# guxm2021/SVT_SpeechBrain

Hardware: AMD Instinct MI355X
Metric: 10s@16kHz clips/sec encoder+CTC forward, wav2vec2-base, 1/2/4/8 MI355X (higher is better)
Workload: dtype bf16; 1 GPU; wav2vec2-base audio-only AMT forward (encoder + 20-way head + frame decode), 32 x 10 s @16 kHz mono clips per GPU; global_batch=32, per_gpu_batch=32, samples_per_clip=160000, frames_per_clip=499, parallelism=clips sharded over 1 rank(s), streams=2, inputs=resident in HBM

## Files before the change

### svt_speechbrain_amd/csrc/api.hip

```cpp
#include "../../include/svt_mi355.h"
#include "api.h"
#include "common.h"
#include "host.h"

#include <atomic>
#include <cmath>
#include <cstring>
#include <map>
#include <mutex>
#include <string>
#include <vector>

namespace svt {

int hip_fail(hipError_t e, const char* what, const char* file, int line) {
  set_error(std::string("HIP error ") + hipGetErrorName(e) + " (" + hipGetErrorString(e) + ") at " + file + ":" +
          std::to_string(line) + " in " + what);
  return SVT_ERR_HIP;
}

struct ProfState {
  bool on = false;
  int every = 1;
  unsigned tick = 0;
// ... 464 lines not shown
  else if (key == 15) g_stamp_ends = value;
  else if (key == 16) {  }
  else if (key == 18) {  }
  else if (key == 19) g_x3_pairs = value;
  else if (key == 20) g_ln_two_rows = value;
  else if (key == 21) {
    if (value != 0 && value != 3) { set_error("svt_debug_set(21): the attention A/B arms are retired"); return SVT_ERR_INVALID; }
  }
  else if (key == 22) g_conv0_mfma = value;
  else if (key == 23) g_conv3x3_c64 = value;
  else if (key == 24) return g_conv3x3_c64_launches;
  else if (key == 25) g_conv3x3_c64_form = value;
  else if (key == 26) g_stem_pool_fused = value;
  else if (key == 27) g_conv_down_fused = value;
  else if (key == 28) {
    if (value != 0) { set_error("svt_debug_set(28): the two-slot schedule is retired"); return SVT_ERR_INVALID; }
  }
  else if (key == 29) g_gemm_p1w = value;
  else if (key == 30) {
#ifndef SVT_DIAG
    if (value != 0) { set_error("svt_debug_set(30): gemm_p1x_kernel is built by `make DIAG=1` only"); return SVT_ERR_INVALID; }
#endif
    g_gemm_p1x = value;
  }
  else if (key == 31) return g_dev_frees.load(std::memory_order_relaxed);
  else if (key == 32) return set_ticket_fenced(value);
  else if (key == 33) g_gemm_skinny_small_tiles = value;
  else if (key == 34) g_gemm_walk = value;
  else if (key == 35) g_conv_kperm = value;
  else if (key == 36) g_ffn2_ksplit = value;
  else if (key == 37) { if (value < 8 || value > 256 || value % 8) { set_error("svt_debug_set(37): 8 .. 256, a multiple of 8"); return SVT_ERR_INVALID; } g_gemm_persist_wgs = value; }
  else if (key == 38) return g_flash_kernel_id;
  else if (key == 39) return g_gemm_kernel_id;
  else { set_error("svt_debug_set: unknown key"); return SVT_ERR_INVALID; }
  return SVT_OK;
}

int svt_debug_alloc(void** out, size_t bytes, int device) {
  if (!out) { set_error("svt_debug_alloc: null argument"); return SVT_ERR_INVALID; }
  if (int r = check_device(device)) return r;
  SVT_HIP(hipSetDevice(device));
  return dev_alloc(out, bytes);
}
int svt_debug_free(void* p, int device) {
  if (int r = check_device(device)) return r;
  SVT_HIP(hipSetDevice(device));
  dev_free(p);
  return SVT_OK;
}

int svt_debug_clock(int64_t* out_dev, int device, void* stream) {
  if (!out_dev) { set_error("svt_debug_clock: null argument"); return SVT_ERR_INVALID; }
  SVT_HIP(hipSetDevice(device));
  return launch_clock_stamp((long long*)out_dev, (hipStream_t)stream) ? SVT_ERR_HIP : SVT_OK;
}

int svt_prof_enable(int on) { g_prof.on = on != 0; g_prof.every = on > 1 ? on : 1; g_prof.tick = 0; return SVT_OK; }
int svt_prof_reset(void) {
  g_prof.used = 0;
  for (int k = 0; k < 3; ++k) g_prof.flops[k] = g_prof.bytes[k] = 0;
  return SVT_OK;
}
int svt_prof_read(int kind, int64_t* launches, double* total_ms, double* total_flops, double* total_bytes) {
  if (kind < 0 || kind > 2) { set_error("svt_prof_read: kind must be 0..2"); return SVT_ERR_INVALID; }
  double ms = 0;
  int64_t n = 0;
// ... 17 lines not shown
```

### svt_speechbrain_amd/csrc/api_encoder.hip

```cpp
#include "../../include/svt_mi355.h"
#include "api.h"
#include "common.h"
#include "host.h"

#include <cmath>
#include <cstring>
#include <string>
#include <vector>

using namespace svt;

int svt::g_conv_ln_bf16 = 1;

struct ConvLayerW {
  DevBuf w;
  DevBuf w_kperm;
  DevBuf bias;
  DevBuf gamma, beta;
};
struct EncLayerW {
  DevBuf wqkv, bqkv, wo, bo, ln1g, ln1b, w1, b1, w2, b2, ln2g, ln2b;
  DevBuf g_wab, g_bab, g_const;
};

struct svt_encoder {
  svt_encoder_config cfg;
  int device = 0;
  bool finalized = false;
  bool uploaded = false;
  ParamMap params;
  std::vector<ConvLayerW> conv;
  DevBuf fp_g, fp_b, proj_w, proj_b, pos_w, pos_b, enc_g, enc_b;
  DevBuf pos_bn_sc, pos_bn_sh;
  DevBuf pos_wP, pos_bP;
  int pos_P = 0;
  std::vector<DevBuf> pos_ws, pos_bs;
  DevBuf rel_embed;
  DevBuf ones, zeros;
  std::vector<EncLayerW> layers;
  svt_norm_reduce_fn reduce_fn = nullptr;
  void* reduce_user = nullptr;
  int64_t reduce_global_clips = 0;
};

static bool reduced_mode(const svt_encoder_config& c) { return c.precision != SVT_PREC_FP32; }
// ... 595 lines not shown
  const svt_encoder_config& c = x.c;
  const EncWs& w = x.w;
  const int C = x.p.C, D = x.p.D, rows = (int)x.p.rows, pk = x.pk_front;
  const void* proj_in = w.act[cur];
  if (c.feat_proj_layer_norm) {
    LnArgs n = ln_f32(x, w.act[cur], rows, C, x.e->fp_g, x.e->fp_b, c.layer_norm_eps);
    n.x_is_f32 = x.p.sp ? 0 : 1;
    (pk ? n.yP : n.yT) = w.xln; n.pair_kind = pk;
    if (int r = launch_layernorm(n, x.s)) return r;
    proj_in = w.xln;
  }
  GemmArgs g;
  g.A = proj_in; g.W = x.e->proj_w.p; g.C = w.hF; g.bias = x.e->proj_b.as<float>();
  g.M = rows; g.N = D; g.K = C; g.a_rpb = rows; g.a_rstride = C; g.ldw = C; g.ldc = D; g.out_f32 = 1;
  g.a_pairs = pk ? 1 : 0;
  return launch_gemm(x.p.gp, g, x.s);
}

GemmArgs posconv_gemm(const EncRun& x, const DevBuf& W, const DevBuf& bias) {
  const int T = (int)x.p.T, D = x.p.D, G = x.c.pos_conv_groups, cg = D / G, kp = x.c.pos_conv_kernel;
  GemmArgs g;
  g.A = x.w.posg; g.W = W.p; g.C = x.w.preF; g.bias = bias.as<float>();
  g.M = T; g.N = cg; g.K = kp * cg;
  g.a_rpb = T; g.a_rstride = cg;
  g.ldw = g.K; g.ldc = D;
  g.nz = x.p.B * G; g.nz2 = G;
  g.a_z1 = (long)G * (T + kp) * cg; g.a_z2 = (long)(T + kp) * cg;
  g.w_z1 = 0; g.w_z2 = (long)cg * g.K;
  g.c_z1 = (long)T * D; g.c_z2 = cg; g.bias_z2 = cg;
  g.out_f32 = 1;
  return g;
}

int positional_conv(const EncRun& x) {
  const svt_encoder_config& c = x.c;
  const svt_encoder* e = x.e;
  const EncWs& w = x.w;
  const int prec = x.p.sp, gp = x.p.gp, B = x.p.B, T = (int)x.p.T, D = x.p.D, kp = c.pos_conv_kernel, G = c.pos_conv_groups, cg = D / G;
  const float* bn_sc = c.pos_conv_batch_norm ? e->pos_bn_sc.as<float>() : nullptr;
  const float* bn_sh = c.pos_conv_batch_norm ? e->pos_bn_sh.as<float>() : nullptr;
  if (c.pos_conv_depth > 1) {
    const float* cur = w.hF;
    float* lnout = w.xF;
    for (int i = 0; i < c.pos_conv_depth; ++i) {
      if (int r = launch_posconv_gather(prec, cur, B, T, D, G, kp, T + kp, w.posg, x.s)) return r;
      GemmArgs g = posconv_gemm(x, e->pos_ws[i], e->pos_bs[i]);
      g.act = ACT_NONE;
      if (int r = launch_gemm(gp, g, x.s)) return r;
      LnArgs n = ln_f32(x, w.preF, x.p.rows, D, e->ones, e->zeros, 1e-5f);
      n.gelu = 1; n.yF = lnout;
      if (int r = launch_layernorm(n, x.s)) return r;
      cur = lnout;
    }
    return launch_add_f32(w.hF, cur, w.preF, x.p.rows * (int64_t)D, x.s);
  }
  if (x.p.pos_multi) {
    const int Pf = x.p.Pf, Tq = (int)x.p.pos_Tq, Tp = (int)x.p.pos_Tp;
    if (int r = launch_posconv_gather(prec, w.hF, B, T, D, G, kp, Tp, w.posg, x.s, bn_sc, bn_sh)) return r;
    GemmArgs g;
    g.A = w.posg; g.W = e->pos_wP.p; g.C = w.posy; g.bias = e->pos_bP.as<float>();
    g.M = B * Tq; g.N = Pf * cg; g.K = (kp + Pf - 1) * cg;
    g.a_rpb = Tq; g.a_bstride = (long)G * Tp * cg; g.a_rstride = (long)Pf * cg;
    g.ldw = g.K; g.ldc = g.N;
    g.nz = G; g.nz2 = G;
    g.a_z2 = (long)Tp * cg; g.w_z2 = (long)g.N * g.K; g.c_z2 = (long)B * Tq * g.N; g.bias_z2 = g.N;
    g.act = ACT_GELU; g.out_f32 = 0;
    if (int r = launch_gemm(gp, g, x.s)) return r;
    return launch_posconv_scatter_add(w.hF, w.posy, B, T, D, G, Pf, Tq, w.preF, x.s, prec ? 0 : 1);
  }
  if (int r = launch_posconv_gather(prec, w.hF, B, T, D, G, kp, T + kp, w.posg, x.s, bn_sc, bn_sh)) return r;
  GemmArgs g = posconv_gemm(x, e->pos_w, e->pos_b);
  g.resid = w.hF; g.act = ACT_GELU;
  return launch_gemm(gp, g, x.s);
}

struct LayerForm {
  int branch_f32 = 1;
  int ffn1_f32 = 0;
  int ffn1_pairs = 0;
  bool ffn2_ksplit = false;
};

int rows_gemm(const EncRun& x, const void* A, int K, const DevBuf& W, const DevBuf& bias, int N, void* Cout, int out_f32, int act,
              unsigned short* planes = nullptr, int c_pairs = 0) {
  const int rows = (int)x.p.rows;
  GemmArgs g;
  g.A = A; g.W = W.p; g.C = Cout; g.bias = bias.as<float>();
  g.M = rows; g.N = N; g.K = K; g.a_rpb = rows; g.a_rstride = K; g.ldw = K; g.ldc = N;
  g.out_f32 = out_f32; g.act = act;
  g.planes = planes; g.plane_stride = (long)rows * N;
  g.a_pairs = x.pk_enc ? 1 : 0; g.c_pairs = c_pairs;
  return launch_gemm(x.p.gp, g, x.s);
}

int attention_block(const EncRun& x, const EncLayerW& Lw, const LayerForm& f) {
  const EncPlan& p = x.p;
  const EncWs& w = x.w;
  const int D = p.D;
  if (int r = rows_gemm(x, w.xb, D, Lw.wqkv, Lw.bqkv, 3 * D, w.qkv, 0, ACT_NONE, p.planes ? (unsigned short*)w.ab.pl_qkv : nullptr)) return r;
  const float* gate = nullptr;
// ... 21 lines not shown

template <class Ln0, class Ln>
int post_ln_layers(const EncRun& x, const LayerForm& f, Ln0&& ln0, Ln&& ln) {
  if (int r = ln0()) return r;
  for (int l = 0; l < x.c.num_layers; ++l) {
    const EncLayerW& Lw = x.e->layers[l];
    if (int r = attention_block(x, Lw, f)) return r;
    if (int r = ln(Lw, false, false)) return r;
    if (int r = ffn_block(x, Lw, f)) return r;
    if (int r = ln(Lw, true, l + 1 == x.c.num_layers)) return r;
  }
  return SVT_OK;
}

bool ffn2_ksplit_ok(const EncRun& x) {
  const int D = x.p.D, F = x.p.F, rows = (int)x.p.rows;
  if (!(g_ffn2_ksplit && x.w.ksplit && x.p.gp == 1 && F % 256 == 0 && F >= 2048 && g_ln_two_rows)) return false;
  GemmArgs g;
  g.A = x.w.ffn; g.W = x.e->layers[0].w2.p; g.C = x.w.hF; g.M = rows; g.N = D; g.K = F; g.a_rpb = rows; g.a_rstride = F; g.ldw = F; g.ldc = D;
  return g_gemm_skinny && gemm_skinny_eligible(g) && (long)((x.p.rows + 31) / 32) * (D / 32) <= 256;
}

int post_ln_hilo(const EncRun& x) {
  const EncWs& w = x.w;
  const int64_t rows = x.p.rows;
  const int D = x.p.D;
  const float eps = x.c.layer_norm_eps;
  bf16_t* const xh = (bf16_t*)w.xb;
  bf16_t* const xl = (bf16_t*)w.xlo;
  LayerForm f;
  f.branch_f32 = 0;
  f.ffn2_ksplit = ffn2_ksplit_ok(x);
  return post_ln_layers(x, f,
    [&] { return launch_layernorm_hilo(nullptr, nullptr, nullptr, w.preF, rows, D, x.e->enc_g.as<float>(), x.e->enc_b.as<float>(), eps, xh, xl, nullptr, x.s); },
    [&](const EncLayerW& Lw, bool second, bool last) {
      const float *g = (second ? Lw.ln2g : Lw.ln1g).as<float>(), *b = (second ? Lw.ln2b : Lw.ln1b).as<float>();
      float* const yF = last ? x.resid : nullptr;
      if (second && f.ffn2_ksplit)
        return launch_layernorm_hilo_parts(w.ksplit, 4, (long)rows * D, Lw.b2.as<float>(), xh, xl, rows, D, g, b, eps, xh, xl, yF, x.s);
      return launch_layernorm_hilo((const bf16_t*)w.hF, xh, xl, nullptr, rows, D, g, b, eps, xh, xl, yF, x.s);
    });
}

int post_ln_pairs(const EncRun& x) {
  const EncWs& w = x.w;
  const bool pair_resid = x.pk_enc == 3;
  LayerForm f;
  f.branch_f32 = 1; f.ffn1_f32 = 1; f.ffn1_pairs = 1;
  return post_ln_layers(x, f,
    [&] {
      LnArgs n = ln_f32(x, w.preF, x.p.rows, x.p.D, x.e->enc_g, x.e->enc_b, x.c.layer_norm_eps);
      n.yP = w.xb; n.pair_kind = x.pk_enc; n.yF = pair_resid ? nullptr : x.resid;
      return launch_layernorm(n, x.s);
    },
    [&](const EncLayerW& Lw, bool second, bool last) {
      LnArgs n = ln_f32(x, w.hF, x.p.rows, x.p.D, second ? Lw.ln2g : Lw.ln1g, second ? Lw.ln2b : Lw.ln1b, x.c.layer_norm_eps);
      n.yP = w.xb; n.pair_kind = x.pk_enc;
      if (pair_resid) { n.addP = w.xb; n.yF = last ? x.resid : nullptr; }
      else { n.add = x.resid; n.yF = x.resid; }
      return launch_layernorm(n, x.s);
    });
}

int post_ln_plain(const EncRun& x, int branch_f32) {
  const EncWs& w = x.w;
  LayerForm f;
  f.branch_f32 = branch_f32;
  auto out = [&](LnArgs n) { n.yT = w.xb; n.yF = x.p.sp ? x.resid : nullptr; return launch_layernorm(n, x.s); };
  return post_ln_layers(x, f,
    [&] { return out(ln_f32(x, w.preF, x.p.rows, x.p.D, x.e->enc_g, x.e->enc_b, x.c.layer_norm_eps)); },
    [&](const EncLayerW& Lw, bool second, bool) {
      LnArgs n = ln_f32(x, w.hF, x.p.rows, x.p.D, second ? Lw.ln2g : Lw.ln1g, second ? Lw.ln2b : Lw.ln1b, x.c.layer_norm_eps);
      n.x_is_f32 = branch_f32; n.add = x.resid;
// ... 137 lines not shown
```

### svt_speechbrain_amd/csrc/common.h

```cpp
#pragma once
#include <hip/hip_runtime.h>
#include <stdint.h>
#include <string>

typedef __bf16 real_bf16x8 __attribute__((ext_vector_type(8)));
#ifdef SVT_OPERAND_F16
typedef _Float16 bf16_t;
#define SVT_MFMA_16x16x32(a, b, c) __builtin_amdgcn_mfma_f32_16x16x32_f16(a, b, c, 0, 0, 0)
#define SVT_MFMA_32x32x16(a, b, c) __builtin_amdgcn_mfma_f32_32x32x16_f16(a, b, c, 0, 0, 0)
#else
typedef __bf16 bf16_t;
#define SVT_MFMA_16x16x32(a, b, c) __builtin_amdgcn_mfma_f32_16x16x32_bf16(a, b, c, 0, 0, 0)
#define SVT_MFMA_32x32x16(a, b, c) __builtin_amdgcn_mfma_f32_32x32x16_bf16(a, b, c, 0, 0, 0)
#endif
typedef bf16_t bf16x8 __attribute__((ext_vector_type(8)));
typedef bf16_t bf16x4 __attribute__((ext_vector_type(4)));
typedef float f32x4 __attribute__((ext_vector_type(4)));

namespace svt {

#if defined(__HIPCC__)
__device__ __forceinline__ float gelu_fast(float x) {
  const float z = fabsf(x) * 0.70710678118654752440f;
  const float t = __builtin_amdgcn_rcpf(fmaf(0.3275911f, z, 1.0f));
// ... 210 lines not shown

__device__ __forceinline__ void tile_walk(int logical, int tiles_m, int tiles_n, int pm, int& tile_m, int& tile_n) {
  if (pm <= 0) { tile_n = logical % tiles_n; tile_m = logical / tiles_n; return; }
  const int per_panel = pm * tiles_n;
  const int pnl = logical / per_panel, rem = logical - pnl * per_panel;
  const int rows = min(pm, tiles_m - pnl * pm);
  tile_n = rem / rows;
  tile_m = pnl * pm + (rem - tile_n * rows);
}

extern int g_gemm_dbg;
extern int g_gemm_force_bm;
extern int g_gemm_ring;
extern int g_gemm_variant;
extern int g_gemm_skinny;
extern int g_gemm_skinny_max_tiles;
extern int g_gemm_x3;
extern int g_stamp_ends;
extern int g_x3_pairs;
extern int g_gemm_p1w;
extern int g_gemm_p1x;
extern int g_gemm_skinny_small_tiles;
extern int g_gemm_walk;
extern int g_conv_kperm;
extern int g_gemm_persist_wgs;
extern int g_gemm_kernel_id;

extern int g_ln_two_rows;
extern int g_flash_wide;
extern int g_flash_kernel_id;
extern int g_ffn2_ksplit;
#pragma GCC visibility push(hidden)
extern int g_conv_ln_bf16;
extern int g_debug_keep_split;
extern int g_conv_down_fused;
#pragma GCC visibility pop

int ensure_dyn_lds(const void* kernel, int bytes);

int dev_alloc(void** out, size_t bytes);
void dev_free(void* p);
extern int g_guard_alloc;

void prof_begin(hipStream_t s);
void prof_end(hipStream_t s, double flops, double bytes, int kind = 1);

int set_ticket_fenced(int on);
int launch_moments(const float* x, int64_t n, double* moments, void* scratch, int groups_max, hipStream_t s, int groups = 1);
size_t moments_scratch_bytes(int groups_max);
int launch_global_norm(const float* x, float* y, int64_t n, const double* moments, float eps, hipStream_t s, int groups = 1,
                       double n_stat = 0);
int launch_conv0_window_moments(const float* wav, int B, int64_t L, int k, int stride, int64_t T1,
                                double* wm , void* scratch , hipStream_t s);
size_t conv0_window_moments_scratch_bytes(int B, int64_t T1);
int launch_conv0_group_coef(const double* wav_moments , int64_t n_wav, const double* wm, int B,
                            int64_t T1, int C, int k, const float* w0 , const float* b0 ,
                            const float* gamma, const float* beta, float eps_wav, float eps_gn,
                            float* coef , hipStream_t s, int clips_per_norm_group);
struct FrameOut { float p_on, p_off; int32_t octave, pitch_class; };
int launch_head_fused(const float* x, int64_t rows, int K, const float* w, const float* wsum, const float* b, int N, float* dots,
                      double* mom, int64_t rows_per_group, float eps, float* logits, FrameOut* frames, int n_oct, int n_cls,
                      hipStream_t s,
                      double n_stat = 0, int (*between)(void*) = nullptr, void* between_arg = nullptr, void* scratch = nullptr);
size_t head_scratch_bytes(int64_t rows, int groups_max);

struct LnArgs {
  int prec = 0;
  const void* x = nullptr;
  int x_is_f32 = 1;
  int64_t rows = 0;
  int D = 0;
  const float* gamma = nullptr;
  const float* beta = nullptr;
  float eps = 1e-5f;
  int gelu = 0;
  void* yT = nullptr;
  float* yF = nullptr;
  const float* add = nullptr;
  float* sumF = nullptr;
  void* yP = nullptr;
  int pair_kind = 0;
  const void* addP = nullptr;
};
int launch_layernorm(const LnArgs& a, hipStream_t s);
bool layernorm_hilo_ok(int D);
int launch_layernorm_hilo_parts(const float* parts, int nparts, long part_stride, const float* pbias, const bf16_t* rh, const bf16_t* rl, int64_t rows,
                                int D, const float* gamma, const float* beta, float eps, bf16_t* yh, bf16_t* yl, float* yF, hipStream_t s);
int launch_layernorm_hilo(const bf16_t* branch, const bf16_t* rh, const bf16_t* rl, const float* x32, int64_t rows, int D,
                          const float* gamma, const float* beta, float eps, bf16_t* yh, bf16_t* yl, float* yF, hipStream_t s);

int launch_conv0_group_apply(int prec, const float* wav, int B, int64_t L, int k, int stride, int64_t T1, int C,
                             const float* coef, void* out , hipStream_t s, int pair_kind = 0);
int launch_conv0_layer(int prec, const float* wav, int B, int64_t L, int k, int stride, int64_t T1, int C,
                       const double* wav_moments, int64_t n_wav, float eps_wav, const float* w0, const float* b0,
                       const float* gamma, const float* beta, float eps, void* out, hipStream_t s, int clips_per_norm_group,
                       int pair_kind = 0);
int launch_f32_to_pairs(int kind, const float* x, void* out, int64_t n, hipStream_t s);
int launch_pairs_to_f32(int kind, const void* in, const void* lo_plane, float* y, int64_t n, hipStream_t s);

bool conv0_mfma_ok(int prec, int pair_kind, int k, int stride, int C);
size_t conv0_mfma_table_bytes(int B);
int launch_conv0_mfma_group(const float* wav, int B, int64_t L, int stride, int64_t T1, const float* coef, void* table_ws, void* out,
                            hipStream_t s, int pair_kind = 0);
int launch_conv0_mfma_layer(const float* wav, int B, int64_t L, int stride, int64_t T1, const double* wav_moments, int64_t n_wav,
                            float eps_wav, const float* w0, const float* b0, const float* gamma, const float* beta, float eps, void* table_ws,
                            void* out, hipStream_t s, int clips_per_norm_group, int pair_kind = 0);
extern int g_conv0_mfma;

int launch_f32_to_bf16(const float* in, bf16_t* out, int64_t n, hipStream_t s);
int launch_zero_bytes(void* p, size_t bytes, hipStream_t s);
int launch_copy_f32(const float* in, float* out, int64_t n, hipStream_t s);
int launch_zero_cols(float* p, int64_t rows, int cols, int64_t ld, hipStream_t s);
int launch_posconv_gather(int prec, const float* h, int B, int T, int D, int G, int kp, int Tp, void* out, hipStream_t s,
                          const float* sc = nullptr, const float* sh = nullptr);
int launch_posconv_scatter_add(const float* h, const void* y, int B, int T, int D, int G, int P, int Tq, float* pre, hipStream_t s,
                               int y_f32 = 0);
int launch_softmax_rows(int prec, const float* S, int64_t rows, int T, int Tp, void* P, hipStream_t s);
int launch_transpose_v(int prec, const void* qkv, int B, int T, int H, int dh, long ld, long voff, int Tp,
                       void* Vt, hipStream_t s);
int launch_axpby(int prec, const void* x, const void* y, float a, float b, void* out, int64_t n, hipStream_t s);
int launch_add_pe(int prec, const float* x, int B, int T, int Tsrc, int D, const float* pe, float* outF, void* outT,
                  hipStream_t s);
// ... 127 lines not shown
```

### svt_speechbrain_amd/csrc/conv0_mfma.hip

```cpp
#include "common.h"

namespace svt {
namespace {

constexpr int K0 = 10, C0 = 512, TBL16 = 2048;

template <int PK> struct C0T { typedef bf16_t piece; };
template <> struct C0T<2> { typedef __bf16 piece; };
template <> struct C0T<3> { typedef _Float16 piece; };
template <int PK> __device__ __forceinline__ f32x4 c0_mma(const typename C0T<PK>::piece __attribute__((ext_vector_type(8))) & a, const uint4& b, const f32x4& c) {
  typedef typename C0T<PK>::piece P;
  typedef P P8 __attribute__((ext_vector_type(8)));
  if constexpr (PK == 3) return __builtin_amdgcn_mfma_f32_16x16x32_f16(a, __builtin_bit_cast(P8, b), c, 0, 0, 0);
  else if constexpr (PK == 2) return __builtin_amdgcn_mfma_f32_16x16x32_bf16(a, __builtin_bit_cast(P8, b), c, 0, 0, 0);
  else return SVT_MFMA_16x16x32(a, __builtin_bit_cast(P8, b), c);
}
template <int PK> __device__ __forceinline__ void c0_store8(void* out, int64_t e, f32x2_t (&p)[4]) {
  typedef typename C0T<PK>::piece P;
  typedef P P8 __attribute__((ext_vector_type(8)));
  if constexpr (PK == 0) {
    gelu_bf16x2_x4(p);
    P8 o;
#pragma unroll
    for (int i = 0; i < 4; ++i) { o[2 * i] = (P)p[i].x; o[2 * i + 1] = (P)p[i].y; }
    *(P8*)((P*)out + e) = o;
  } else {
    P8 hi, lo;
#pragma unroll
    for (int i = 0; i < 4; ++i) {
      const f32x2_t y = gelu_fast2(p[i]);
      hi[2 * i] = (P)y.x; lo[2 * i] = (P)(y.x - (float)hi[2 * i]);
      hi[2 * i + 1] = (P)y.y; lo[2 * i + 1] = (P)(y.y - (float)hi[2 * i + 1]);
    }
    char* d = (char*)out + (e >> 5) * 128 + (e & 31) * 2;
    *(P8*)d = hi;
    *(P8*)(d + 64) = lo;
  }
}

__global__ __launch_bounds__(256) void conv0_coef_exp_kernel(const float* __restrict__ coef, int* __restrict__ exps) {
  const int b = blockIdx.x;
  float mx = 0.f;
  for (int i = threadIdx.x; i < C0 * K0; i += 256) mx = fmaxf(mx, fabsf(coef[((long)b * C0 + i / K0) * (K0 + 1) + i % K0]));
#pragma unroll
  for (int o = 32; o > 0; o >>= 1) mx = fmaxf(mx, __shfl_xor(mx, o, 64));
  __shared__ float part[4];
  if ((threadIdx.x & 63) == 0) part[threadIdx.x >> 6] = mx;
  __syncthreads();
  if (threadIdx.x == 0) {
    mx = fmaxf(fmaxf(part[0], part[1]), fmaxf(part[2], part[3]));
    int e = 0;
    if (mx > 0.f && mx < 3e38f) (void)frexpf(mx, &e);
    exps[b] = e > 100 ? 100 : (e < -100 ? -100 : e);
  }
}

template <int PK>
__global__ void conv0_table_kernel(const float* __restrict__ w, long w_clip_stride, int w_row, const float* __restrict__ bias,
                                   void* __restrict__ table_, const int* __restrict__ tap_exp) {
  typedef typename C0T<PK>::piece bf16_t;
  typedef bf16_t bf16x8 __attribute__((ext_vector_type(8)));
  bf16_t* table = (bf16_t*)table_;
  const int b = blockIdx.y;
  const int idx = blockIdx.x * blockDim.x + threadIdx.x;
  if (idx >= TBL16) return;
  const int blk = idx >> 6, lane = idx & 63, q = blk >> 3, nb = blk & 7, g = lane >> 4, j = lane & 15;
  const int c = 128 * q + 8 * j + nb;
  const float* wc = w + (long)b * w_clip_stride + (long)c * w_row;
  const float bv = bias ? bias[c] : (w_row == K0 + 1 ? wc[K0] : 0.f);
  const float tap_scale = tap_exp ? ldexpf(1.f, -tap_exp[b]) : 1.f;
  bf16x8 o;
#pragma unroll
  for (int i = 0; i < 8; ++i) {
    const int k = 8 * g + i;
    const float src = k < 30 ? wc[k % 10] * tap_scale : bv;
    const bf16_t hi = (bf16_t)src;
    const bf16_t lo = (bf16_t)(src - (float)hi);
    o[i] = (k < 20 || k == 30) ? hi : lo;
  }
  *(bf16x8*)(table + ((long)b * TBL16 + idx) * 8) = o;
}

template <int MODE, int PK = 0>
__global__ __launch_bounds__(256) void conv0_mfma_kernel(const float* __restrict__ wav, int64_t L, int stride, int64_t T1,
                                                         const void* __restrict__ table_, long table_clip_stride,
                                                         const double* __restrict__ wav_mom, int64_t n_wav, float eps_wav,
                                                         const float* __restrict__ gamma, const float* __restrict__ beta, float eps, int cpg,
                                                         void* __restrict__ out, const int* __restrict__ tap_exp) {
  typedef typename C0T<PK>::piece bf16_t;
  typedef bf16_t bf16x8 __attribute__((ext_vector_type(8)));
  const bf16_t* table = (const bf16_t*)table_;
  constexpr int FPW = 64;
  __shared__ __attribute__((aligned(16))) uint4 tbl[TBL16];
  __shared__ float xs[4][FPW * 5 + 16];
  const int tid = threadIdx.x, lane = tid & 63, wave = tid >> 6;
  const int b = blockIdx.y;
  {
    const uint4* tg = (const uint4*)(table + (long)b * table_clip_stride);
    for (int i = tid; i < TBL16; i += 256) tbl[i] = tg[i];
  }
  float mu = 0.f, rn = 1.f, xscale = 1.f, bscale = 1.f;
  if (MODE == 1 && wav_mom) {
    const double* wm = wav_mom + 2 * (b / cpg);
// ... 89 lines not shown
      }
#pragma unroll
      for (int r = 0; r < 4; ++r) {
        float qq = 0.f;
#pragma unroll
        for (int blk = 0; blk < 32; ++blk) { const float d = acc[blk][r] - mean[r]; qq = fmaf(d, d, qq); }
#pragma unroll
        for (int o = 8; o > 0; o >>= 1) qq += __shfl_xor(qq, o, 64);
        rstd[r] = rsqrtf(qq * (1.f / C0) + eps);
      }
#pragma unroll
      for (int q = 0; q < 4; ++q) {
        __builtin_amdgcn_sched_barrier(0);
        const float4 g0 = *(const float4*)(gamma + 128 * q + 8 * j), g1 = *(const float4*)(gamma + 128 * q + 8 * j + 4);
        const float4 b0 = *(const float4*)(beta + 128 * q + 8 * j), b1 = *(const float4*)(beta + 128 * q + 8 * j + 4);
        const float gg[8] = {g0.x, g0.y, g0.z, g0.w, g1.x, g1.y, g1.z, g1.w}, bb[8] = {b0.x, b0.y, b0.z, b0.w, b1.x, b1.y, b1.z, b1.w};
#pragma unroll
        for (int r = 0; r < 4; ++r) {
          f32x2_t p[4];
#pragma unroll
          for (int i = 0; i < 4; ++i)
            p[i] = f32x2_t{fmaf((acc[q * 8 + 2 * i][r] - mean[r]) * rstd[r], gg[2 * i], bb[2 * i]),
                           fmaf((acc[q * 8 + 2 * i + 1][r] - mean[r]) * rstd[r], gg[2 * i + 1], bb[2 * i + 1])};
          if (fr0 + r < nfr) c0_store8<PK>(out, e0 + (int64_t)r * C0 + 128 * q, p);
        }
      }
    }
  }
}

}

int g_conv0_mfma = 1;

bool conv0_mfma_ok(int prec, int pair_kind, int k, int stride, int C) {
  return g_conv0_mfma && (prec == 1 || pair_kind == 2 || pair_kind == 3) && k == K0 && stride >= 1 && stride <= 5 && C == C0;
}
size_t conv0_mfma_table_bytes(int B) { return (size_t)B * TBL16 * 16 + (((size_t)B * 4 + 255) & ~(size_t)255); }

#define SVT_C0_DISPATCH(PKV, STMT)                 \
  if ((PKV) == 3) { constexpr int PK_ = 3; STMT }  \
  else if ((PKV) == 2) { constexpr int PK_ = 2; STMT } \
  else { constexpr int PK_ = 0; STMT }

int launch_conv0_mfma_group(const float* wav, int B, int64_t L, int stride, int64_t T1, const float* coef, void* table_ws, void* out,
                            hipStream_t s, int pair_kind) {
  if (((uintptr_t)table_ws & 15) || ((uintptr_t)out & 127)) { set_error("conv0_mfma: alignment"); return -1; }
  dim3 grid((unsigned)((T1 + 255) / 256), B);
  int* exps = (int*)((char*)table_ws + (size_t)B * TBL16 * 16);
  hipLaunchKernelGGL(conv0_coef_exp_kernel, dim3(B), dim3(256), 0, s, coef, exps);
  SVT_C0_DISPATCH(pair_kind,
    hipLaunchKernelGGL((conv0_table_kernel<PK_>), dim3(TBL16 / 256, B), dim3(256), 0, s, coef, (long)C0 * (K0 + 1), K0 + 1, (const float*)nullptr,
                       table_ws, (const int*)exps);
    hipLaunchKernelGGL((conv0_mfma_kernel<0, PK_>), grid, dim3(256), 0, s, wav, L, stride, T1, (const void*)table_ws, (long)TBL16 * 8,
                       (const double*)nullptr, (int64_t)1, 0.f, (const float*)nullptr, (const float*)nullptr, 0.f, 1, out, (const int*)exps);)
  SVT_LAUNCH_CHECK();
  return 0;
}

int launch_conv0_mfma_layer(const float* wav, int B, int64_t L, int stride, int64_t T1, const double* wav_moments, int64_t n_wav,
                            float eps_wav, const float* w0, const float* b0, const float* gamma, const float* beta, float eps, void* table_ws,
                            void* out, hipStream_t s, int cpg, int pair_kind) {
  if (((uintptr_t)table_ws & 15) || ((uintptr_t)out & 127) || ((uintptr_t)gamma & 15) || ((uintptr_t)beta & 15)) { set_error("conv0_mfma: alignment"); return -1; }
  dim3 grid((unsigned)((T1 + 255) / 256), B);
  SVT_C0_DISPATCH(pair_kind,
    hipLaunchKernelGGL((conv0_table_kernel<PK_>), dim3(TBL16 / 256, 1), dim3(256), 0, s, w0, 0L, K0, b0, table_ws, (const int*)nullptr);
    hipLaunchKernelGGL((conv0_mfma_kernel<1, PK_>), grid, dim3(256), 0, s, wav, L, stride, T1, (const void*)table_ws, 0L, wav_moments, n_wav,
                       eps_wav, gamma, beta, eps, cpg, out, (const int*)nullptr);)
  SVT_LAUNCH_CHECK();
  return 0;
}
#undef SVT_C0_DISPATCH

}
```

### svt_speechbrain_amd/csrc/layernorm.hip

```cpp
#include "device_util.h"
#include <type_traits>

namespace svt {
namespace {
template <typename TI, typename TO>
__global__ __launch_bounds__(256) void layernorm_kernel(const TI* x, const float* add, float* sumF, int64_t rows, int D,
                                                        const float* gamma, const float* beta, float eps, int gelu,
                                                        TO* yT, float* yF) {
  const int lane = threadIdx.x & 63;
  const int64_t row = (int64_t)blockIdx.x * 4 + (threadIdx.x >> 6);
  if (row >= rows) return;
  const TI* xr = x + row * D;
  const float* ar = add ? add + row * D : nullptr;
  float s = 0.f;
  for (int i = lane; i < D; i += 64) s += ld<TI>(xr, i) + (ar ? ar[i] : 0.f);
  const float mean = wave_sum(s) / (float)D;
  float q = 0.f;
  for (int i = lane; i < D; i += 64) { const float d = ld<TI>(xr, i) + (ar ? ar[i] : 0.f) - mean; q += d * d; }
  const float rstd = rsqrtf(wave_sum(q) / (float)D + eps);
  for (int i = lane; i < D; i += 64) {
    const float xv = ld<TI>(xr, i) + (ar ? ar[i] : 0.f);
    if (sumF) sumF[row * D + i] = xv;
    float v = (xv - mean) * rstd * gamma[i] + beta[i];
    if (gelu) v = gelu_erf(v);
// ... 187 lines not shown
                                                             bf16_t* yh, bf16_t* yl, float* yF) {
  constexpr int D = 64 * VPT, NV = VPT / 4;
  const int lane = threadIdx.x & 63;
  const int64_t row = (int64_t)blockIdx.x * 4 + (threadIdx.x >> 6);
  if (row >= rows) return;
  float v[VPT];
  float s = 0.f;
#pragma unroll
  for (int j = 0; j < NV; ++j) {
    const long o = row * D + (lane + 64 * j) * 4;
    const bf16x4 h = *(const bf16x4*)(rh + o), l = *(const bf16x4*)(rl + o);
    float4 t = float4{(float)h[0] + (float)l[0], (float)h[1] + (float)l[1], (float)h[2] + (float)l[2], (float)h[3] + (float)l[3]};
    if (branch) {
      const bf16x4 a = *(const bf16x4*)(branch + o);
      t.x += (float)a[0]; t.y += (float)a[1]; t.z += (float)a[2]; t.w += (float)a[3];
    }
    v[4 * j] = t.x; v[4 * j + 1] = t.y; v[4 * j + 2] = t.z; v[4 * j + 3] = t.w;
    s += (t.x + t.y) + (t.z + t.w);
  }
  const float mean = wave_sum(s) * (1.f / D);
  float q = 0.f;
#pragma unroll
  for (int i = 0; i < VPT; ++i) { v[i] -= mean; q = fmaf(v[i], v[i], q); }
  const float rstd = rsqrtf(wave_sum(q) * (1.f / D) + eps);
#pragma unroll
  for (int j = 0; j < NV; ++j) {
    const int c = (lane + 64 * j) * 4;
    const float4 g = *(const float4*)(gamma + c), b = *(const float4*)(beta + c);
    const float o[4] = {fmaf(v[4 * j] * rstd, g.x, b.x), fmaf(v[4 * j + 1] * rstd, g.y, b.y),
                        fmaf(v[4 * j + 2] * rstd, g.z, b.z), fmaf(v[4 * j + 3] * rstd, g.w, b.w)};
    bf16x4 oh, ol;
#pragma unroll
    for (int i = 0; i < 4; ++i) { oh[i] = (bf16_t)o[i]; ol[i] = (bf16_t)(o[i] - (float)oh[i]); }
    *(bf16x4*)(yh + row * D + c) = oh;
    *(bf16x4*)(yl + row * D + c) = ol;
    if (yF) *(float4*)(yF + row * D + c) = float4{o[0], o[1], o[2], o[3]};
  }
}

template <int D, bool PARTS = false>
__global__ __launch_bounds__(256) void layernorm_hilo2_kernel(const bf16_t* branch, const bf16_t* rh, const bf16_t* rl,
                                                              int64_t rows, const float* gamma, const float* beta, float eps,
                                                              bf16_t* yh, bf16_t* yl, float* yF, const float* parts = nullptr, int nparts = 0,
                                                              long part_stride = 0, const float* pbias = nullptr) {
  constexpr int NC = D / 256;
  const int lane = threadIdx.x & 63, sub = lane & 31;
  const int64_t row = (int64_t)blockIdx.x * 8 + (threadIdx.x >> 6) * 2 + (lane >> 5);
  if (row >= rows) return;
  float v[NC][8];
  float s = 0.f;
#pragma unroll
  for (int j = 0; j < NC; ++j) {
    const long o = row * D + (sub + 32 * j) * 8;
    const bf16x8 h = *(const bf16x8*)(rh + o), l = *(const bf16x8*)(rl + o);
#pragma unroll
    for (int i = 0; i < 8; ++i) v[j][i] = (float)h[i] + (float)l[i];
    if constexpr (PARTS) {
      float a[8];
      {
        const float4 t0 = *(const float4*)(parts + o), t1 = *(const float4*)(parts + o + 4);
        a[0] = t0.x; a[1] = t0.y; a[2] = t0.z; a[3] = t0.w; a[4] = t1.x; a[5] = t1.y; a[6] = t1.z; a[7] = t1.w;
      }
      for (int k = 1; k < nparts; ++k) {
        const float4 t0 = *(const float4*)(parts + k * part_stride + o), t1 = *(const float4*)(parts + k * part_stride + o + 4);
        a[0] += t0.x; a[1] += t0.y; a[2] += t0.z; a[3] += t0.w; a[4] += t1.x; a[5] += t1.y; a[6] += t1.z; a[7] += t1.w;
      }
      const int c = (sub + 32 * j) * 8;
      const float4 b0 = *(const float4*)(pbias + c), b1 = *(const float4*)(pbias + c + 4);
// ... 2 lines not shown
      for (int i = 0; i < 8; ++i) v[j][i] += (float)(bf16_t)(a[i] + bb[i]);
    } else if (branch) {
      const bf16x8 a = *(const bf16x8*)(branch + o);
#pragma unroll
      for (int i = 0; i < 8; ++i) v[j][i] += (float)a[i];
    }
    s += ((v[j][0] + v[j][1]) + (v[j][2] + v[j][3])) + ((v[j][4] + v[j][5]) + (v[j][6] + v[j][7]));
  }
#pragma unroll
  for (int o = 16; o > 0; o >>= 1) s += __shfl_xor(s, o, 64);
  const float mean = s * (1.f / D);
  float q = 0.f;
#pragma unroll
  for (int j = 0; j < NC; ++j)
#pragma unroll
    for (int i = 0; i < 8; ++i) { v[j][i] -= mean; q = fmaf(v[j][i], v[j][i], q); }
#pragma unroll
  for (int o = 16; o > 0; o >>= 1) q += __shfl_xor(q, o, 64);
  const float rstd = rsqrtf(q * (1.f / D) + eps);
#pragma unroll
  for (int j = 0; j < NC; ++j) {
    const int c = (sub + 32 * j) * 8;
    const float4 g0 = *(const float4*)(gamma + c), g1 = *(const float4*)(gamma + c + 4);
    const float4 b0 = *(const float4*)(beta + c), b1 = *(const float4*)(beta + c + 4);
    const float gg[8] = {g0.x, g0.y, g0.z, g0.w, g1.x, g1.y, g1.z, g1.w}, bb[8] = {b0.x, b0.y, b0.z, b0.w, b1.x, b1.y, b1.z, b1.w};
    float o[8];
    bf16x8 oh, ol;
#pragma unroll
    for (int i = 0; i < 8; ++i) {
      o[i] = fmaf(v[j][i] * rstd, gg[i], bb[i]);
      oh[i] = (bf16_t)o[i];
      ol[i] = (bf16_t)(o[i] - (float)oh[i]);
    }
    *(bf16x8*)(yh + row * D + c) = oh;
    *(bf16x8*)(yl + row * D + c) = ol;
    if (yF) {
      *(float4*)(yF + row * D + c) = float4{o[0], o[1], o[2], o[3]};
      *(float4*)(yF + row * D + c + 4) = float4{o[4], o[5], o[6], o[7]};
    }
  }
}
template <int VPT>
__global__ __launch_bounds__(256) void layernorm_f32_to_hilo_kernel(const float* x, int64_t rows, const float* gamma,
                                                                    const float* beta, float eps, bf16_t* yh, bf16_t* yl) {
  constexpr int D = 64 * VPT, NV = VPT / 4;
  const int lane = threadIdx.x & 63;
  const int64_t row = (int64_t)blockIdx.x * 4 + (threadIdx.x >> 6);
  if (row >= rows) return;
  float v[VPT];
  float s = 0.f;
#pragma unroll
  for (int j = 0; j < NV; ++j) {
    const float4 t = ((const float4*)(x + row * D))[lane + 64 * j];
    v[4 * j] = t.x; v[4 * j + 1] = t.y; v[4 * j + 2] = t.z; v[4 * j + 3] = t.w;
    s += (t.x + t.y) + (t.z + t.w);
  }
  const float mean = wave_sum(s) * (1.f / D);
  float q = 0.f;
#pragma unroll
  for (int i = 0; i < VPT; ++i) { v[i] -= mean; q = fmaf(v[i], v[i], q); }
  const float rstd = rsqrtf(wave_sum(q) * (1.f / D) + eps);
#pragma unroll
  for (int j = 0; j < NV; ++j) {
    const int c = (lane + 64 * j) * 4;
    const float4 g = *(const float4*)(gamma + c), b = *(const float4*)(beta + c);
    const float o[4] = {fmaf(v[4 * j] * rstd, g.x, b.x), fmaf(v[4 * j + 1] * rstd, g.y, b.y),
                        fmaf(v[4 * j + 2] * rstd, g.z, b.z), fmaf(v[4 * j + 3] * rstd, g.w, b.w)};
    bf16x4 oh, ol;
#pragma unroll
    for (int i = 0; i < 4; ++i) { oh[i] = (bf16_t)o[i]; ol[i] = (bf16_t)(o[i] - (float)oh[i]); }
    *(bf16x4*)(yh + row * D + c) = oh;
    *(bf16x4*)(yl + row * D + c) = ol;
  }
}
}
bool layernorm_hilo_ok(int D) { return D == 512 || D == 768 || D == 1024; }
int launch_layernorm_hilo_parts(const float* parts, int nparts, long part_stride, const float* pbias, const bf16_t* rh, const bf16_t* rl, int64_t rows,
                                int D, const float* gamma, const float* beta, float eps, bf16_t* yh, bf16_t* yl, float* yF, hipStream_t s) {
  if (!parts || nparts < 1 || !pbias || !(D == 512 || D == 768 || D == 1024) || (part_stride & 3) || !aligned(15, parts, pbias, rh, rl, yh, yl, yF, gamma, beta)) { set_error("layernorm (K-split branch): D in {512, 768, 1024} and 16-byte aligned buffers"); return -1; }
  const dim3 grid2((unsigned)((rows + 7) / 8)), block(256);
  ln_width(D, [&](auto vpt) {
    hipLaunchKernelGGL((layernorm_hilo2_kernel<64 * decltype(vpt)::value, true>), grid2, block, 0, s, nullptr, rh, rl, rows, gamma, beta, eps, yh, yl, yF, parts, nparts, part_stride, pbias);
  });
  SVT_LAUNCH_CHECK();
  return 0;
}
int launch_layernorm_hilo(const bf16_t* branch, const bf16_t* rh, const bf16_t* rl, const float* x32, int64_t rows, int D,
                          const float* gamma, const float* beta, float eps, bf16_t* yh, bf16_t* yl, float* yF, hipStream_t s) {
  const dim3 grid((unsigned)((rows + 3) / 4)), grid2((unsigned)((rows + 7) / 8)), block(256);
  ln_width(D, [&](auto vpt) {
    constexpr int VPT = decltype(vpt)::value;
    if (x32) hipLaunchKernelGGL((layernorm_f32_to_hilo_kernel<VPT>), grid, block, 0, s, x32, rows, gamma, beta, eps, yh, yl);
    else if (g_ln_two_rows && aligned(15, branch, rh, rl, yh, yl, yF, gamma, beta)) hipLaunchKernelGGL((layernorm_hilo2_kernel<64 * VPT>), grid2, block, 0, s, branch, rh, rl, rows, gamma, beta, eps, yh, yl, yF);
    else hipLaunchKernelGGL((layernorm_hilo_kernel<VPT>), grid, block, 0, s, branch, rh, rl, rows, gamma, beta, eps, yh, yl, yF);
  });
  SVT_LAUNCH_CHECK();
  return 0;
}

}
```

Measured before the change: 6315 clips/s.

## Fuse posconv scatter-add into first LayerNorm, skip last-layer planes, fold conv0 exponent

The positional-conv scatter-add and the encoder's first LayerNorm now run as one kernel that reads the residual and the grouped conv output directly, so the fp32 intermediate no longer round-trips through memory. The last encoder LayerNorm can now write only its fp32 result and skip the unused bf16 hi/lo planes. The conv0 per-clip exponent reduction is folded into the table kernel, removing one launch. Each block of the table kernel recomputes the max reduction, which adds some redundant work, and debug counters are added.

```diff
diff --git a/svt_speechbrain_amd/csrc/api.hip b/svt_speechbrain_amd/csrc/api.hip
--- a/svt_speechbrain_amd/csrc/api.hip
+++ b/svt_speechbrain_amd/csrc/api.hip
@@ -520,6 +520,10 @@
   else if (key == 37) { if (value < 8 || value > 256 || value % 8) { set_error("svt_debug_set(37): 8 .. 256, a multiple of 8"); return SVT_ERR_INVALID; } g_gemm_persist_wgs = value; }
   else if (key == 38) return g_flash_kernel_id;
   else if (key == 39) return g_gemm_kernel_id;
+  else if (key == 40) g_posconv_ln_fused = value;
+  else if (key == 41) g_last_ln_f32_only = value;
+  else if (key == 42) g_conv0_self_exp = value;
+  else if (key == 43) { if (value < 0 || value > 2) { set_error("svt_debug_set(43): 0 .. 2"); return SVT_ERR_INVALID; } return g_seam_runs[value]; }
   else { set_error("svt_debug_set: unknown key"); return SVT_ERR_INVALID; }
   return SVT_OK;
 }
diff --git a/svt_speechbrain_amd/csrc/api_encoder.hip b/svt_speechbrain_amd/csrc/api_encoder.hip
--- a/svt_speechbrain_amd/csrc/api_encoder.hip
+++ b/svt_speechbrain_amd/csrc/api_encoder.hip
@@ -11,6 +11,9 @@
 using namespace svt;
 
 int svt::g_conv_ln_bf16 = 1;
+int svt::g_posconv_ln_fused = 1;
+int svt::g_last_ln_f32_only = 1;
+int svt::g_seam_runs[3] = {0, 0, 0};
 
 struct ConvLayerW {
   DevBuf w;
@@ -672,6 +675,13 @@
   return g;
 }
 
+bool posconv_ln_fused(const EncRun& x) {
+  const EncWs& w = x.w;
+  return g_posconv_ln_fused && x.p.hilo && x.p.sp && x.p.pos_multi && x.c.pos_conv_depth <= 1 &&
+         posconv_add_layernorm_hilo_ok(x.p.D, x.c.pos_conv_groups, w.hF, w.posy, x.e->enc_g.as<float>(), x.e->enc_b.as<float>(),
+                                       (const bf16_t*)w.xb, (const bf16_t*)w.xlo);
+}
+
 int positional_conv(const EncRun& x) {
   const svt_encoder_config& c = x.c;
   const svt_encoder* e = x.e;
@@ -706,6 +716,7 @@
     g.a_z2 = (long)Tp * cg; g.w_z2 = (long)g.N * g.K; g.c_z2 = (long)B * Tq * g.N; g.bias_z2 = g.N;
     g.act = ACT_GELU; g.out_f32 = 0;
     if (int r = launch_gemm(gp, g, x.s)) return r;
+    if (posconv_ln_fused(x)) return SVT_OK;
     return launch_posconv_scatter_add(w.hF, w.posy, B, T, D, G, Pf, Tq, w.preF, x.s, prec ? 0 : 1);
   }
   if (int r = launch_posconv_gather(prec, w.hF, B, T, D, G, kp, T + kp, w.posg, x.s, bn_sc, bn_sh)) return r;
@@ -793,13 +804,23 @@
   f.branch_f32 = 0;
   f.ffn2_ksplit = ffn2_ksplit_ok(x);
   return post_ln_layers(x, f,
-    [&] { return launch_layernorm_hilo(nullptr, nullptr, nullptr, w.preF, rows, D, x.e->enc_g.as<float>(), x.e->enc_b.as<float>(), eps, xh, xl, nullptr, x.s); },
+    [&] {
+      if (posconv_ln_fused(x)) {
+        ++g_seam_runs[0];
+        return launch_posconv_add_layernorm_hilo(w.hF, (const bf16_t*)w.posy, x.p.B, (int)x.p.T, D, x.c.pos_conv_groups, x.p.Pf, (int)x.p.pos_Tq,
+                                                 x.e->enc_g.as<float>(), x.e->enc_b.as<float>(), eps, xh, xl, x.s);
+      }
+      return launch_layernorm_hilo(nullptr, nullptr, nullptr, w.preF, rows, D, x.e->enc_g.as<float>(), x.e->enc_b.as<float>(), eps, xh, xl, nullptr, x.s);
+    },
     [&](const EncLayerW& Lw, bool second, bool last) {
       const float *g = (second ? Lw.ln2g : Lw.ln1g).as<float>(), *b = (second ? Lw.ln2b : Lw.ln1b).as<float>();
       float* const yF = last ? x.resid : nullptr;
+      const bool planes = !(last && g_last_ln_f32_only);
+      if (!planes) ++g_seam_runs[1];
+      bf16_t *const yh = planes ? xh : nullptr, *const yl = planes ? xl : nullptr;
       if (second && f.ffn2_ksplit)
-        return launch_layernorm_hilo_parts(w.ksplit, 4, (long)rows * D, Lw.b2.as<float>(), xh, xl, rows, D, g, b, eps, xh, xl, yF, x.s);
-      return launch_layernorm_hilo((const bf16_t*)w.hF, xh, xl, nullptr, rows, D, g, b, eps, xh, xl, yF, x.s);
+        return launch_layernorm_hilo_parts(w.ksplit, 4, (long)rows * D, Lw.b2.as<float>(), xh, xl, rows, D, g, b, eps, yh, yl, yF, x.s);
+      return launch_layernorm_hilo((const bf16_t*)w.hF, xh, xl, nullptr, rows, D, g, b, eps, yh, yl, yF, x.s);
     });
 }
 
diff --git a/svt_speechbrain_amd/csrc/common.h b/svt_speechbrain_amd/csrc/common.h
--- a/svt_speechbrain_amd/csrc/common.h
+++ b/svt_speechbrain_amd/csrc/common.h
@@ -266,6 +266,10 @@
 extern int g_ffn2_ksplit;
 #pragma GCC visibility push(hidden)
 extern int g_conv_ln_bf16;
+extern int g_posconv_ln_fused;
+extern int g_last_ln_f32_only;
+extern int g_conv0_self_exp;
+extern int g_seam_runs[3];
 extern int g_debug_keep_split;
 extern int g_conv_down_fused;
 #pragma GCC visibility pop
@@ -322,6 +326,9 @@
                                 int D, const float* gamma, const float* beta, float eps, bf16_t* yh, bf16_t* yl, float* yF, hipStream_t s);
 int launch_layernorm_hilo(const bf16_t* branch, const bf16_t* rh, const bf16_t* rl, const float* x32, int64_t rows, int D,
                           const float* gamma, const float* beta, float eps, bf16_t* yh, bf16_t* yl, float* yF, hipStream_t s);
+bool posconv_add_layernorm_hilo_ok(int D, int G, const float* h, const void* y, const float* gamma, const float* beta, const bf16_t* yh, const bf16_t* yl);
+int launch_posconv_add_layernorm_hilo(const float* h, const bf16_t* y, int B, int T, int D, int G, int P, int Tq, const float* gamma,
+                                      const float* beta, float eps, bf16_t* yh, bf16_t* yl, hipStream_t s);
 
 int launch_conv0_group_apply(int prec, const float* wav, int B, int64_t L, int k, int stride, int64_t T1, int C,
                              const float* coef, void* out , hipStream_t s, int pair_kind = 0);
diff --git a/svt_speechbrain_amd/csrc/conv0_mfma.hip b/svt_speechbrain_amd/csrc/conv0_mfma.hip
--- a/svt_speechbrain_amd/csrc/conv0_mfma.hip
+++ b/svt_speechbrain_amd/csrc/conv0_mfma.hip
@@ -38,6 +38,11 @@
   }
 }
 
+__device__ __forceinline__ int conv0_tap_exp(float mx) {
+  int e = 0;
+  if (mx > 0.f && mx < 3e38f) (void)frexpf(mx, &e);
+  return e > 100 ? 100 : (e < -100 ? -100 : e);
+}
 __global__ __launch_bounds__(256) void conv0_coef_exp_kernel(const float* __restrict__ coef, int* __restrict__ exps) {
   const int b = blockIdx.x;
   float mx = 0.f;
@@ -47,28 +52,35 @@
   __shared__ float part[4];
   if ((threadIdx.x & 63) == 0) part[threadIdx.x >> 6] = mx;
   __syncthreads();
-  if (threadIdx.x == 0) {
-    mx = fmaxf(fmaxf(part[0], part[1]), fmaxf(part[2], part[3]));
-    int e = 0;
-    if (mx > 0.f && mx < 3e38f) (void)frexpf(mx, &e);
-    exps[b] = e > 100 ? 100 : (e < -100 ? -100 : e);
-  }
+  if (threadIdx.x == 0) exps[b] = conv0_tap_exp(fmaxf(fmaxf(part[0], part[1]), fmaxf(part[2], part[3])));
 }
 
 template <int PK>
 __global__ void conv0_table_kernel(const float* __restrict__ w, long w_clip_stride, int w_row, const float* __restrict__ bias,
-                                   void* __restrict__ table_, const int* __restrict__ tap_exp) {
+                                   void* __restrict__ table_, const int* __restrict__ tap_exp, int* __restrict__ exp_out) {
   typedef typename C0T<PK>::piece bf16_t;
   typedef bf16_t bf16x8 __attribute__((ext_vector_type(8)));
   bf16_t* table = (bf16_t*)table_;
   const int b = blockIdx.y;
+  int own_exp = 0;
+  if (exp_out) {
+    float mx = 0.f;
+    for (int i = threadIdx.x; i < C0 * K0; i += 256) mx = fmaxf(mx, fabsf(w[(long)b * w_clip_stride + (long)(i / K0) * w_row + i % K0]));
+#pragma unroll
+    for (int o = 32; o > 0; o >>= 1) mx = fmaxf(mx, __shfl_xor(mx, o, 64));
+    __shared__ float part[4];
+    if ((threadIdx.x & 63) == 0) part[threadIdx.x >> 6] = mx;
+    __syncthreads();
+    own_exp = conv0_tap_exp(fmaxf(fmaxf(part[0], part[1]), fmaxf(part[2], part[3])));
+    if (blockIdx.x == 0 && threadIdx.x == 0) exp_out[b] = own_exp;
+  }
   const int idx = blockIdx.x * blockDim.x + threadIdx.x;
   if (idx >= TBL16) return;
   const int blk = idx >> 6, lane = idx & 63, q = blk >> 3, nb = blk & 7, g = lane >> 4, j = lane & 15;
   const int c = 128 * q + 8 * j + nb;
   const float* wc = w + (long)b * w_clip_stride + (long)c * w_row;
   const float bv = bias ? bias[c] : (w_row == K0 + 1 ? wc[K0] : 0.f);
-  const float tap_scale = tap_exp ? ldexpf(1.f, -tap_exp[b]) : 1.f;
+  const float tap_scale = exp_out ? ldexpf(1.f, -own_exp) : (tap_exp ? ldexpf(1.f, -tap_exp[b]) : 1.f);
   bf16x8 o;
 #pragma unroll
   for (int i = 0; i < 8; ++i) {
@@ -224,6 +236,7 @@
 }
 
 int g_conv0_mfma = 1;
+int g_conv0_self_exp = 1;
 
 bool conv0_mfma_ok(int prec, int pair_kind, int k, int stride, int C) {
   return g_conv0_mfma && (prec == 1 || pair_kind == 2 || pair_kind == 3) && k == K0 && stride >= 1 && stride <= 5 && C == C0;
@@ -240,10 +253,12 @@
   if (((uintptr_t)table_ws & 15) || ((uintptr_t)out & 127)) { set_error("conv0_mfma: alignment"); return -1; }
   dim3 grid((unsigned)((T1 + 255) / 256), B);
   int* exps = (int*)((char*)table_ws + (size_t)B * TBL16 * 16);
-  hipLaunchKernelGGL(conv0_coef_exp_kernel, dim3(B), dim3(256), 0, s, coef, exps);
+  const bool self_exp = g_conv0_self_exp && pair_kind == 0;
+  if (self_exp) ++g_seam_runs[2];
+  else hipLaunchKernelGGL(conv0_coef_exp_kernel, dim3(B), dim3(256), 0, s, coef, exps);
   SVT_C0_DISPATCH(pair_kind,
     hipLaunchKernelGGL((conv0_table_kernel<PK_>), dim3(TBL16 / 256, B), dim3(256), 0, s, coef, (long)C0 * (K0 + 1), K0 + 1, (const float*)nullptr,
-                       table_ws, (const int*)exps);
+                       table_ws, self_exp ? (const int*)nullptr : (const int*)exps, self_exp ? exps : (int*)nullptr);
     hipLaunchKernelGGL((conv0_mfma_kernel<0, PK_>), grid, dim3(256), 0, s, wav, L, stride, T1, (const void*)table_ws, (long)TBL16 * 8,
                        (const double*)nullptr, (int64_t)1, 0.f, (const float*)nullptr, (const float*)nullptr, 0.f, 1, out, (const int*)exps);)
   SVT_LAUNCH_CHECK();
@@ -256,7 +271,7 @@
   if (((uintptr_t)table_ws & 15) || ((uintptr_t)out & 127) || ((uintptr_t)gamma & 15) || ((uintptr_t)beta & 15)) { set_error("conv0_mfma: alignment"); return -1; }
   dim3 grid((unsigned)((T1 + 255) / 256), B);
   SVT_C0_DISPATCH(pair_kind,
-    hipLaunchKernelGGL((conv0_table_kernel<PK_>), dim3(TBL16 / 256, 1), dim3(256), 0, s, w0, 0L, K0, b0, table_ws, (const int*)nullptr);
+    hipLaunchKernelGGL((conv0_table_kernel<PK_>), dim3(TBL16 / 256, 1), dim3(256), 0, s, w0, 0L, K0, b0, table_ws, (const int*)nullptr, (int*)nullptr);
     hipLaunchKernelGGL((conv0_mfma_kernel<1, PK_>), grid, dim3(256), 0, s, wav, L, stride, T1, (const void*)table_ws, 0L, wav_moments, n_wav,
                        eps_wav, gamma, beta, eps, cpg, out, (const int*)nullptr);)
   SVT_LAUNCH_CHECK();
diff --git a/svt_speechbrain_amd/csrc/layernorm.hip b/svt_speechbrain_amd/csrc/layernorm.hip
--- a/svt_speechbrain_amd/csrc/layernorm.hip
+++ b/svt_speechbrain_amd/csrc/layernorm.hip
@@ -243,8 +243,10 @@
     bf16x4 oh, ol;
 #pragma unroll
     for (int i = 0; i < 4; ++i) { oh[i] = (bf16_t)o[i]; ol[i] = (bf16_t)(o[i] - (float)oh[i]); }
-    *(bf16x4*)(yh + row * D + c) = oh;
-    *(bf16x4*)(yl + row * D + c) = ol;
+    if (yh) {
+      *(bf16x4*)(yh + row * D + c) = oh;
+      *(bf16x4*)(yl + row * D + c) = ol;
+    }
     if (yF) *(float4*)(yF + row * D + c) = float4{o[0], o[1], o[2], o[3]};
   }
 }
@@ -313,12 +315,36 @@
       oh[i] = (bf16_t)o[i];
       ol[i] = (bf16_t)(o[i] - (float)oh[i]);
     }
-    *(bf16x8*)(yh + row * D + c) = oh;
-    *(bf16x8*)(yl + row * D + c) = ol;
+    if (yh) {
+      *(bf16x8*)(yh + row * D + c) = oh;
+      *(bf16x8*)(yl + row * D + c) = ol;
+    }
     if (yF) {
       *(float4*)(yF + row * D + c) = float4{o[0], o[1], o[2], o[3]};
       *(float4*)(yF + row * D + c + 4) = float4{o[4], o[5], o[6], o[7]};
     }
+  }
+}
+template <int VPT>
+__device__ __forceinline__ void row_f32_to_hilo(float (&v)[VPT], float s, int64_t row, int lane, const float* gamma, const float* beta,
+                                                float eps, bf16_t* yh, bf16_t* yl) {
+  constexpr int D = 64 * VPT, NV = VPT / 4;
+  const float mean = wave_sum(s) * (1.f / D);
+  float q = 0.f;
+#pragma unroll
+  for (int i = 0; i < VPT; ++i) { v[i] -= mean; q = fmaf(v[i], v[i], q); }
+  const float rstd = rsqrtf(wave_sum(q) * (1.f / D) + eps);
+#pragma unroll
+  for (int j = 0; j < NV; ++j) {
+    const int c = (lane + 64 * j) * 4;
+    const float4 g = *(const float4*)(gamma + c), b = *(const float4*)(beta + c);
+    const float o[4] = {fmaf(v[4 * j] * rstd, g.x, b.x), fmaf(v[4 * j + 1] * rstd, g.y, b.y),
+                        fmaf(v[4 * j + 2] * rstd, g.z, b.z), fmaf(v[4 * j + 3] * rstd, g.w, b.w)};
+    bf16x4 oh, ol;
+#pragma unroll
+    for (int i = 0; i < 4; ++i) { oh[i] = (bf16_t)o[i]; ol[i] = (bf16_t)(o[i] - (float)oh[i]); }
+    *(bf16x4*)(yh + row * D + c) = oh;
+    *(bf16x4*)(yl + row * D + c) = ol;
   }
 }
 template <int VPT>
@@ -336,29 +362,40 @@
     v[4 * j] = t.x; v[4 * j + 1] = t.y; v[4 * j + 2] = t.z; v[4 * j + 3] = t.w;
     s += (t.x + t.y) + (t.z + t.w);
   }
-  const float mean = wave_sum(s) * (1.f / D);
-  float q = 0.f;
-#pragma unroll
-  for (int i = 0; i < VPT; ++i) { v[i] -= mean; q = fmaf(v[i], v[i], q); }
-  const float rstd = rsqrtf(wave_sum(q) * (1.f / D) + eps);
-#pragma unroll
-  for (int j = 0; j < NV; ++j) {
-    const int c = (lane + 64 * j) * 4;
-    const float4 g = *(const float4*)(gamma + c), b = *(const float4*)(beta + c);
-    const float o[4] = {fmaf(v[4 * j] * rstd, g.x, b.x), fmaf(v[4 * j + 1] * rstd, g.y, b.y),
-                        fmaf(v[4 * j + 2] * rstd, g.z, b.z), fmaf(v[4 * j + 3] * rstd, g.w, b.w)};
-    bf16x4 oh, ol;
-#pragma unroll
-    for (int i = 0; i < 4; ++i) { oh[i] = (bf16_t)o[i]; ol[i] = (bf16_t)(o[i] - (float)oh[i]); }
-    *(bf16x4*)(yh + row * D + c) = oh;
-    *(bf16x4*)(yl + row * D + c) = ol;
-  }
+  row_f32_to_hilo<VPT>(v, s, row, lane, gamma, beta, eps, yh, yl);
+}
+template <int VPT>
+__global__ __launch_bounds__(256) void posconv_add_layernorm_to_hilo_kernel(const float* h, const bf16_t* y, int B, int T, int G, int P, int Tq,
+                                                                            const float* gamma, const float* beta, float eps, bf16_t* yh,
+                                                                            bf16_t* yl) {
+  constexpr int D = 64 * VPT, NV = VPT / 4;
+  const int lane = threadIdx.x & 63;
+  const int64_t rows = (int64_t)B * T;
+  const int64_t row = (int64_t)blockIdx.x * 4 + (threadIdx.x >> 6);
+  if (row >= rows) return;
+  const int cg = D / G;
+  const int t = (int)(row % T), b = (int)(row / T);
+  const int q = t / P, jf = t - q * P;
+  float v[VPT];
+  float s = 0.f;
+#pragma unroll
+  for (int j = 0; j < NV; ++j) {
+    const int ch = (lane + 64 * j) * 4;
+    const int g = ch / cg, c = ch - g * cg;
+    const bf16x4 a = *(const bf16x4*)(y + (((int64_t)g * B + b) * Tq + q) * (P * cg) + jf * cg + c);
+    const float4 hv = ((const float4*)(h + row * D))[lane + 64 * j];
+    const float4 t4 = float4{hv.x + (float)a[0], hv.y + (float)a[1], hv.z + (float)a[2], hv.w + (float)a[3]};
+    v[4 * j] = t4.x; v[4 * j + 1] = t4.y; v[4 * j + 2] = t4.z; v[4 * j + 3] = t4.w;
+    s += (t4.x + t4.y) + (t4.z + t4.w);
+  }
+  row_f32_to_hilo<VPT>(v, s, row, lane, gamma, beta, eps, yh, yl);
 }
 }
 bool layernorm_hilo_ok(int D) { return D == 512 || D == 768 || D == 1024; }
 int launch_layernorm_hilo_parts(const float* parts, int nparts, long part_stride, const float* pbias, const bf16_t* rh, const bf16_t* rl, int64_t rows,
                                 int D, const float* gamma, const float* beta, float eps, bf16_t* yh, bf16_t* yl, float* yF, hipStream_t s) {
   if (!parts || nparts < 1 || !pbias || !(D == 512 || D == 768 || D == 1024) || (part_stride & 3) || !aligned(15, parts, pbias, rh, rl, yh, yl, yF, gamma, beta)) { set_error("layernorm (K-split branch): D in {512, 768, 1024} and 16-byte aligned buffers"); return -1; }
+  if (!yh != !yl || (!yh && !yF)) { set_error("layernorm (hi, lo): the planes come as a pair; without them the fp32 result is the output"); return -1; }
   const dim3 grid2((unsigned)((rows + 7) / 8)), block(256);
   ln_width(D, [&](auto vpt) {
     hipLaunchKernelGGL((layernorm_hilo2_kernel<64 * decltype(vpt)::value, true>), grid2, block, 0, s, nullptr, rh, rl, rows, gamma, beta, eps, yh, yl, yF, parts, nparts, part_stride, pbias);
@@ -368,6 +405,7 @@
 }
 int launch_layernorm_hilo(const bf16_t* branch, const bf16_t* rh, const bf16_t* rl, const float* x32, int64_t rows, int D,
                           const float* gamma, const float* beta, float eps, bf16_t* yh, bf16_t* yl, float* yF, hipStream_t s) {
+  if (!yh != !yl || (!yh && (x32 || !yF))) { set_error("layernorm (hi, lo): the planes come as a pair; without them the fp32 result is the output"); return -1; }
   const dim3 grid((unsigned)((rows + 3) / 4)), grid2((unsigned)((rows + 7) / 8)), block(256);
   ln_width(D, [&](auto vpt) {
     constexpr int VPT = decltype(vpt)::value;
@@ -378,5 +416,18 @@
   SVT_LAUNCH_CHECK();
   return 0;
 }
-
-}
+bool posconv_add_layernorm_hilo_ok(int D, int G, const float* h, const void* y, const float* gamma, const float* beta, const bf16_t* yh, const bf16_t* yl) {
+  return layernorm_hilo_ok(D) && G > 0 && D % G == 0 && (D / G) % 4 == 0 && aligned(15, h, gamma, beta) && aligned(7, y, yh, yl);
+}
+int launch_posconv_add_layernorm_hilo(const float* h, const bf16_t* y, int B, int T, int D, int G, int P, int Tq, const float* gamma,
+                                      const float* beta, float eps, bf16_t* yh, bf16_t* yl, hipStream_t s) {
+  if (!posconv_add_layernorm_hilo_ok(D, G, h, y, gamma, beta, yh, yl) || P < 1 || (int64_t)Tq * P < T) { set_error("layernorm (positional conv + first norm): shape or alignment"); return -1; }
+  const int64_t rows = (int64_t)B * T;
+  ln_width(D, [&](auto vpt) {
+    hipLaunchKernelGGL((posconv_add_layernorm_to_hilo_kernel<decltype(vpt)::value>), dim3((unsigned)((rows + 3) / 4)), dim3(256), 0, s, h, y, B, T, G, P, Tq, gamma, beta, eps, yh, yl);
+  });
+  SVT_LAUNCH_CHECK();
+  return 0;
+}
+
+}
```

Result: no change. 6344 clips/s, median of 4 (+0.5%).
